# joanrod/star-vector

Measured on AMD Instinct MI355X. Metric: SVG tokens/sec (whole job) + p50 time-to-first-token, StarVector-1B im2svg batch32/GPU, higher is better.
Workload: dtype bf16; 1 GPU; StarVector-1B im2svg, batch 32/GPU, bf16, greedy, 224x224, prompt rows 259 (257 visual + 2), 1024 new tokens/seq, EOS disabled; global_batch=32, parallelism=single, hipgraph_decode=True, decode_steps_per_graph_launch=32, exclusive_device=True

## Files before the change

include/starvector_hip_debug.h:

```cpp
#ifndef STARVECTOR_HIP_DEBUG_H
#define STARVECTOR_HIP_DEBUG_H

#include "starvector_hip.h"

#ifdef __cplusplus
extern "C" {
#endif

int  sv_debug_resample_coeffs(int32_t in_size, int32_t out_size, int32_t* bounds, int32_t* taps, int32_t cap);
int  sv_debug_skinny_plan(int32_t rows, int32_t N, int32_t K, int32_t splitk, int32_t wfmt, int32_t* out2);
enum sv_exp_bits {
    SV_EXP_NO_LN_FOLD        = 2,
    SV_EXP_MLP_FUSED_FORCE   = 128,
    SV_EXP_MLP_FUSED_OFF     = 512,
    SV_EXP_SEPARATE_ARGMAX   = 1024,
    SV_EXP_ROWLN_CATTN_OFF   = 8192,
    SV_EXP_ROWLN_CATTN_FORCE = 16384,
    SV_EXP_NO_PRUNE_LAST     = 32768,
    SV_EXP_BATCH_REMAINDER   = 4194304,
    SV_EXP_KNOWN = SV_EXP_NO_LN_FOLD | SV_EXP_MLP_FUSED_FORCE | SV_EXP_MLP_FUSED_OFF | SV_EXP_SEPARATE_ARGMAX | SV_EXP_ROWLN_CATTN_OFF |
                   SV_EXP_ROWLN_CATTN_FORCE | SV_EXP_NO_PRUNE_LAST | SV_EXP_BATCH_REMAINDER
};
int  sv_debug_set_exp(sv_engine* e, int32_t mask);
int  sv_debug_exp_known(void);
int  sv_debug_gemm_plan(int32_t M, int32_t N, int32_t K, int32_t act, int32_t* out5);
int  sv_debug_decode_plan(int32_t rows, int32_t N, int32_t K, int32_t wfmt, int32_t whole_k, int32_t num_cus, int32_t* out2);
int  sv_debug_attn_plan(int32_t max_batch, int32_t n_kv_head, int32_t num_cus, int32_t* out2);
int  sv_debug_rowln_plan(int32_t D, int32_t N, int32_t splitk, int32_t splitk_ru, int32_t num_cus, int32_t* out3);
int  sv_debug_rowln_occupancy(int32_t wide, int32_t* blocks_per_cu);
int  sv_debug_step_plan(sv_engine* e, int32_t* out4);
int  sv_debug_set_col_tiles(int32_t col_tiles);
int  sv_debug_set_skinny_form(int32_t form);
int  sv_debug_skinny_form(void);
int  sv_debug_tailsplit_launches(int64_t* count);
int  sv_debug_cols_rowhalf_launches(int64_t* launches, int64_t* halves);
int  sv_debug_set_gemm_form(int32_t form);
int  sv_debug_set_linear_seq_rows(int32_t seq_rows);
int  sv_debug_gemm_seq_form(int32_t S, int32_t N, int32_t K, int32_t act);
int  sv_debug_ragged_plan(const int32_t* lens, int32_t B, int32_t N, int32_t K, int32_t act, int32_t q_tile, int32_t* rows_out,
                          int32_t* last_out, int32_t capacity, int32_t* out4);
int  sv_debug_prefix_plan(const int32_t* prefix_lens, int32_t P, const int32_t* lens, const int32_t* prefix_of, int32_t B, int32_t N,
                          int32_t K, int32_t act, int32_t q_tile, int32_t* row_pos_out, int32_t* rows_out, int32_t* blocks_out,
                          int32_t capacity, int32_t* out4);
int  sv_debug_extend_plan(const int32_t* ctx, const int32_t* lens, const int32_t* totals, int32_t B, int32_t budget, int32_t N, int32_t K,
                          int32_t act, int32_t q_tile, int32_t* out, int32_t capacity, int32_t* out_n);
int  sv_debug_shared_plan(const int32_t* lens, int32_t n_prompts, const int32_t* group, const int32_t* budgets, int32_t n,
                          int32_t* shared_out, int32_t* private_out, int64_t* total_out);
int  sv_debug_block_table(sv_engine* e, int32_t row, int32_t* host_out, int32_t capacity);
int  sv_debug_free_pages(sv_engine* e, int32_t* free_out, int32_t* total_out);
int  sv_debug_prompt_passes(sv_engine* e, int64_t* out);
int  sv_debug_attn_trace(sv_engine* e, int64_t* host_out, int32_t capacity_rows);
int  sv_debug_mlp_trace(sv_engine* e, int64_t* host_out, int32_t capacity_blocks);
int  sv_debug_xcc_map(sv_engine* e, int32_t blocks, int32_t heavy, int32_t* host_out);
int  sv_debug_occupy_cus(sv_engine* e, int32_t blocks, int32_t lds_bytes, int32_t ms);
int  sv_debug_gemm_trace(int32_t M, int32_t N, int32_t K, int32_t act, int32_t form, int64_t* host_out, int32_t capacity_blocks);
int  sv_debug_kv_load(sv_engine* e, int32_t layer, const void* dev_kv, int32_t B, int32_t S, const int32_t* dev_lens,
                      sv_stream stream);
int  sv_debug_kv_read(sv_engine* e, int32_t layer, int32_t row, int32_t first, int32_t count, void* dev_out_bf16, sv_stream stream);
int  sv_debug_kv_gather(sv_engine* e, int32_t layer, int32_t row, int32_t count, void* dev_out_bf16, sv_stream stream);
int  sv_debug_page_digests(const void* dev_embeds_packed, int32_t n, const int32_t* host_lens, int32_t S0, int32_t hidden, int32_t max_pages,
                           uint64_t* host_out, sv_stream stream);
int  sv_debug_prefix_hit(const uint64_t* host_digests, int32_t n_pages, int32_t L, const uint64_t* host_table_keys, int32_t n_table,
                         uint64_t* host_keys_out, int32_t* h_out);
int  sv_debug_attn_decode(sv_engine* e, int32_t layer, const float* dev_qkv_f32, int32_t B, void* dev_out, int32_t advance,
                          sv_stream stream);
int  sv_debug_attn_decode_slabs(sv_engine* e, int32_t layer, const float* dev_slabs_f32, int32_t splitk, const void* dev_bias, int32_t B,
                                void* dev_out, int32_t advance, sv_stream stream);
int  sv_debug_attn_decode_draft(sv_engine* e, int32_t layer, const float* dev_slabs_f32, int32_t splitk, const void* dev_bias, int32_t n_seq,
// ... 126 lines not shown
```

star-vector_amd/_lib.py:

```python
from __future__ import annotations

import ctypes as C
import os

HERE = os.path.dirname(os.path.abspath(__file__))
LIB_PATH = os.path.join(HERE, "libstarvector_hip.so")
HEADER_PATH = os.path.normpath(os.path.join(HERE, "..", "include", "starvector_hip.h"))
DEBUG_HEADER_PATH = os.path.normpath(os.path.join(HERE, "..", "include", "starvector_hip_debug.h"))

ABI_VERSION = 9
SV_DTYPE_BF16, SV_DTYPE_F32 = 0, 1
SV_NORM_LAYER, SV_NORM_BATCH = 0, 1
SV_ARCH_V1, SV_ARCH_V2 = 0, 1
ACT = {"none": 0, "quickgelu": 1, "swish": 2, "gelu_tanh": 3}


class SvConfig(C.Structure):
    _fields_ = [
        ("image_size", C.c_int32), ("patch_size", C.c_int32), ("vit_width", C.c_int32),
        ("vit_layers", C.c_int32), ("vit_heads", C.c_int32), ("adapter_norm", C.c_int32),
        ("hidden", C.c_int32), ("n_layer", C.c_int32), ("n_head", C.c_int32), ("n_inner", C.c_int32),
        ("vocab", C.c_int32), ("n_positions", C.c_int32), ("max_batch", C.c_int32),
        ("max_seq_len", C.c_int32), ("ln_eps", C.c_float), ("device", C.c_int32),
        ("arch", C.c_int32), ("n_kv_head", C.c_int32), ("rope_theta", C.c_float), ("vit_mlp", C.c_int32),
# ... 135 lines not shown
    "sv_generate": (_I, [_P, _P, _I, _I, C.POINTER(SvSampling), _P, C.POINTER(_I), _P]),
    "sv_generate_ex": (_I, [_P, _P, _I, _I, C.POINTER(SvSampling), C.POINTER(SvGenerateOutputs), _P, C.POINTER(_I), _P]),
    "sv_cb_admit": (_I, [_P, _P, _I, _I, C.POINTER(SvCbRequest), C.POINTER(_I), _P]),
    "sv_cb_step": (_I, [_P, _I, C.POINTER(_I), _P]),
    "sv_cb_poll": (_I, [_P, C.POINTER(_I), C.POINTER(_I), _I]),
    "sv_cb_read": (_I, [_P, _I, _I, _I, C.POINTER(C.c_int64)]),
    "sv_cb_release": (_I, [_P, _I]),
    "sv_cb_reset": (_I, [_P]),
    "sv_cb_admit_logprobs": (_I, [_P, _P, _I, C.POINTER(_I), _I, C.POINTER(_I), C.POINTER(SvCbRequest), C.POINTER(SvCbLogprobs), C.POINTER(_I), _P]),
    "sv_cb_read_logprobs": (_I, [_P, _I, _I, _I, C.POINTER(_F), C.POINTER(_I), C.POINTER(_I), C.POINTER(_F)]),
    "sv_cb_set_lookup": (_I, [_P, C.POINTER(SvLookup)]),
    "sv_cb_lookup_counts": (_I, [_P, _I, C.POINTER(_I)]),
    "sv_cb_set_prefix_cache": (_I, [_P, _I]),
    "sv_cb_prefix_cache_info": (_I, [_P, C.POINTER(C.c_int64)]),
    "sv_beam_create": (_I, [C.POINTER(SvBeamConfig), C.POINTER(_P)]),
    "sv_beam_destroy": (_I, [_P]),
    "sv_beam_step": (_I, [_P, _P, _I, C.POINTER(_I), C.POINTER(_I), C.POINTER(_I), C.POINTER(_F), _P]),
    "sv_beam_finalize": (_I, [_P, C.POINTER(C.c_int64), C.POINTER(_I), C.POINTER(_F), _P]),
    "sv_beam_history": (_I, [_P, C.POINTER(_I), C.POINTER(_I), _I, C.POINTER(_I), C.POINTER(_I)]),
    "sv_last_timing": (_I, [_P, C.POINTER(C.c_double)]),
}

DEBUG_PROTOTYPES = {
    "sv_debug_resample_coeffs": (_I, [_I, _I, C.POINTER(_I), C.POINTER(_I), _I]),
    "sv_debug_gemm_plan": (_I, [_I, _I, _I, _I, C.POINTER(_I)]),
    "sv_debug_skinny_plan": (_I, [_I, _I, _I, _I, _I, C.POINTER(_I)]),
    "sv_debug_set_exp": (_I, [_P, _I]),
    "sv_debug_exp_known": (_I, []),
    "sv_debug_set_col_tiles": (_I, [_I]),
    "sv_debug_set_skinny_form": (_I, [_I]),
    "sv_debug_skinny_form": (_I, []),
    "sv_debug_tailsplit_launches": (_I, [C.POINTER(C.c_int64)]),
    "sv_debug_cols_rowhalf_launches": (_I, [C.POINTER(C.c_int64), C.POINTER(C.c_int64)]),
    "sv_debug_set_gemm_form": (_I, [_I]),
    "sv_debug_set_linear_seq_rows": (_I, [_I]),
    "sv_debug_gemm_seq_form": (_I, [_I, _I, _I, _I]),
    "sv_debug_ragged_plan": (_I, [C.POINTER(_I), _I, _I, _I, _I, _I, C.POINTER(_I), C.POINTER(_I), _I, C.POINTER(_I)]),
    "sv_debug_prefix_plan": (_I, [C.POINTER(_I), _I, C.POINTER(_I), C.POINTER(_I), _I, _I, _I, _I, _I, C.POINTER(_I), C.POINTER(_I), C.POINTER(_I), _I,
                                  C.POINTER(_I)]),
    "sv_debug_prompt_passes": (_I, [_P, C.POINTER(C.c_int64)]),
    "sv_debug_extend_plan": (_I, [C.POINTER(_I), C.POINTER(_I), C.POINTER(_I), _I, _I, _I, _I, _I, _I, C.POINTER(_I), _I, C.POINTER(_I)]),
    "sv_debug_kv_gather": (_I, [_P, _I, _I, _I, _P, _P]),
    "sv_debug_page_digests": (_I, [_P, _I, C.POINTER(_I), _I, _I, _I, C.POINTER(C.c_uint64), _P]),
    "sv_debug_prefix_hit": (_I, [C.POINTER(C.c_uint64), _I, _I, C.POINTER(C.c_uint64), _I, C.POINTER(C.c_uint64), C.POINTER(_I)]),
    "sv_debug_shared_plan": (_I, [C.POINTER(_I), _I, C.POINTER(_I), C.POINTER(_I), _I, C.POINTER(_I), C.POINTER(_I), C.POINTER(C.c_int64)]),
    "sv_debug_block_table": (_I, [_P, _I, C.POINTER(_I), _I]),
    "sv_debug_free_pages": (_I, [_P, C.POINTER(_I), C.POINTER(_I)]),
    "sv_debug_attn_plan": (_I, [_I, _I, _I, C.POINTER(_I)]),
    "sv_debug_rowln_plan": (_I, [_I, _I, _I, _I, _I, C.POINTER(_I)]),
    "sv_debug_rowln_occupancy": (_I, [_I, C.POINTER(_I)]),
    "sv_debug_step_plan": (_I, [_P, C.POINTER(_I)]),
    "sv_debug_attn_trace": (_I, [_P, C.POINTER(C.c_int64), _I]),
    "sv_debug_mlp_trace": (_I, [_P, C.POINTER(C.c_int64), _I]),
    "sv_debug_xcc_map": (_I, [_P, _I, _I, C.POINTER(_I)]),
    "sv_debug_occupy_cus": (_I, [_P, _I, _I, _I]),
    "sv_debug_gemm_trace": (_I, [_I, _I, _I, _I, _I, C.POINTER(C.c_int64), _I]),
    "sv_debug_kv_load": (_I, [_P, _I, _P, _I, _I, _P, _P]),
    "sv_debug_kv_read": (_I, [_P, _I, _I, _I, _I, _P, _P]),
    "sv_debug_attn_decode": (_I, [_P, _I, _P, _I, _P, _I, _P]),
    "sv_debug_attn_decode_slabs": (_I, [_P, _I, _P, _I, _P, _I, _P, _I, _P]),
    "sv_debug_attn_decode_draft": (_I, [_P, _I, _P, _I, _P, _I, _I, _P, _P]),
    "sv_debug_set_lookup_drafts": (_I, [_P, C.POINTER(_I), _I, _I]),
    "sv_op_lookup_accept": (_I, [C.POINTER(_I), C.POINTER(_I), _I, _I, _I, _I, C.POINTER(_I), _I, C.POINTER(_I), C.POINTER(_I), C.POINTER(_I), _I,
                                 _I, _I, _I, _I, C.POINTER(_I), C.POINTER(_I), _P]),
    "sv_op_lookup_draft": (_I, [C.POINTER(_I), _I, _I, _I, _I, _I, C.POINTER(_I), C.POINTER(_I), _P]),
    "sv_op_lookup_hold": (_I, [_P, _I, _I, _I, _I, _I, C.POINTER(_I), _P]),
# ... 116 lines not shown
```

star-vector_amd/csrc/attention.hip:

```cpp
#include "kernels.h"
#include "kv8/kv8_dev.h"

namespace sv {

__device__ __forceinline__ int swap23(int x) { return (x & ~0xC) | ((x & 4) << 1) | ((x & 8) >> 1); }

template <int D, int HPB, bool RAG = false, bool PFX = false>
__global__ __launch_bounds__(256, 2) void attn_prefill_kernel(AttnPrefillArgs p) {

    constexpr int KSTR = D + 8;
    constexpr int VSTR = 64 + 8;
    constexpr int NKS = D / 16;
    constexpr int NDV = D / 32;
    __shared__ __attribute__((aligned(16))) bf16_t Ks[64 * KSTR];
    __shared__ __attribute__((aligned(16))) bf16_t Vt[D * VSTR];

    const int tid = threadIdx.x, lane = tid & 63;
    const int wave = __builtin_amdgcn_readfirstlane(tid >> 6);
    const int c = lane >> 5;
    int S, qtile;
    size_t row0;
    int pl = 0;
    long long prow = 0, orow = 0;
    if constexpr (PFX) {
// ... 406 lines not shown

template <int D>
struct KvFrags {
    u32x4 k[2][D / 32];
    u32x4 v[D / 16];
};

template <int D>
__device__ __forceinline__ void load_group(KvFrags<D>& f, const char* pool, int page_index, int page_bytes,
                                           int g, int lane) {
    constexpr int NKS = D / 32, NDV = D / 16;
    const int t0 = g << 5;
    const char* page = pool + (size_t)page_index * page_bytes;
    const int half = (t0 >> 5) & 1;
#pragma unroll
    for (int u = 0; u < 2; ++u)
#pragma unroll
        for (int s = 0; s < NKS; ++s)
            f.k[u][s] = *reinterpret_cast<const u32x4*>(page + ((size_t)(((half * 2 + u) * NKS + s) * 64 + lane)) * 16);
#pragma unroll
    for (int t = 0; t < NDV; ++t)
        f.v[t] = *reinterpret_cast<const u32x4*>(page + (size_t)64 * D * 2 + ((size_t)((half * NDV + t) * 64 + lane)) * 16);
}

__device__ __forceinline__ unsigned xcc_id() {
    unsigned x;
    asm volatile("s_getreg_b32 %0, hwreg(HW_REG_XCC_ID)" : "=s"(x));
    return x & 15u;
}

struct AttnDecodeKernarg { const float* ws; const bf16_t* bias; const int32_t* positions; const int32_t* block_table; char* pool_layer;
                           int max_pages; unsigned geom; int ldws; unsigned rows_heads; size_t kv_head_stride; int window;
                           AttnDecodeArgs p; };
template <int D, int NS, int KVF = 0>
__global__ __launch_bounds__(AD_WAVES * 64) void attn_decode_kernel(const float* ws_, const bf16_t* bias_, const int32_t* positions_, const int32_t* block_table_,
                                                                     char* pool_layer_, int max_pages_, unsigned geom_, int ldws_, unsigned rows_heads_,
                                                                     size_t kv_head_stride_, int window_, AttnDecodeArgs p_unused) {
    constexpr int NKS = D / 32;
    constexpr int NDV = D / 16;
    constexpr int PART = 32 + 16 * D;
    const long long t_start = wall_clock64();
    const int n_kv_ = (int)(geom_ & 255u), max_splits_ = (int)((geom_ >> 8) & 255u), gpb_ = (int)((geom_ >> 16) & 255u);
    const int splitk_ = (int)(geom_ >> 24), rows_ws_ = (int)(rows_heads_ & 0xffffu);
    const int H = (int)(rows_heads_ >> 16);
    const int bx = blockIdx.x;
    const int b = bx / n_kv_;
    const int kvh = bx % n_kv_;
    const int split = blockIdx.y;
    const int G = H / n_kv_;
    const int HD = G * D;
    const int tid = threadIdx.x, lane = tid & 63;
    const int wave = __builtin_amdgcn_readfirstlane(tid >> 6);
    const int pos = *reinterpret_cast<const int32_t __attribute__((address_space(4)))*>(reinterpret_cast<uintptr_t>(positions_ + b));

    constexpr int SLT = (AD_WAVES / 2) * 64;
    constexpr int QQ = 16 * D / 4 / SLT;
    static_assert(QQ * SLT * 4 == 16 * D && 2 * D <= SLT && (2 * D & (2 * D - 1)) == 0, "slab work does not tile the upper half of the block");
    const bool slab_wave = wave >= AD_WAVES / 2;
    const unsigned st = (unsigned)tid & (SLT - 1);
    f32x4 sq[QQ][NS];
    float sk[NS];
    uint2 bq[QQ];
    unsigned bk = 0;
    const unsigned kc = st & (2 * D - 1);
    const unsigned kcol = (unsigned)(H * D + kvh * D) + (kc < D ? 0u : (unsigned)(n_kv_ * D)) + (kc & (D - 1));
    auto qcol = [&](int i) -> unsigned {
        const unsigned n = (st + i * SLT) * 4, r = n / D;
// ... 324 lines not shown
                float den = 0.f;
#pragma unroll
                for (int w = 0; w < NWV; ++w) {
                    const float mw = m_s[w * 16 + h];
                    den = fmaf((mw == -INFINITY) ? 0.f : __expf(mw - M), l_s[w * 16 + h], den);
                }
                v[j] = __float_as_uint(is_l ? den : M);
            }
            __builtin_amdgcn_raw_buffer_store_b128(v, rs, my_off + tid * 16, 0, 16);
        }
    };
    if (nwa <= 4) block_merge(std::integral_constant<int, 4>{});
    else if (nwa <= 6) block_merge(std::integral_constant<int, 6>{});
    else block_merge(std::integral_constant<int, AD_WAVES>{});
    auto stamp = [&](long long t_part, long long t_tick, long long t_end) {
        if (p.trace && tid == 0) {
            long long* q = p.trace + ((size_t)bx * gridDim.y + split) * 16;
            q[0] = t_start; q[1] = t_kvreq; q[2] = t_q; q[3] = t_loop; q[4] = t_part; q[5] = t_tick; q[6] = t_end; q[7] = act; q[8] = ngroups;
        }
    };
    if (act == 1) { stamp(0, 0, wall_clock64()); return; }

    asm volatile("s_waitcnt vmcnt(0)" ::: "memory");
    __syncthreads();
    const long long t_part = wall_clock64();
    if (tid == 0) {
        const unsigned t = __hip_atomic_fetch_add(p.counters + bx, 1u, __ATOMIC_RELAXED, __HIP_MEMORY_SCOPE_AGENT);
        flag_s[0] = (t == (unsigned)(act - 1)) ? 1 : 0;
    }
    __syncthreads();
    const long long t_tick = wall_clock64();
    if (!flag_s[0]) { stamp(t_part, t_tick, 0); return; }
    const int seq_off = (int)((size_t)bx * AD_SPLIT * PART * 4);
    for (int idx = tid * 4; idx < HD; idx += AD_WAVES * 64 * 4) {
        const int h = idx / D;
        u32x4 ov[AD_SPLIT];
        float ms[AD_SPLIT], ls[AD_SPLIT];
#pragma unroll
        for (int s2 = 0; s2 < AD_SPLIT; ++s2) {
            ov[s2] = u32x4{0u, 0u, 0u, 0u};
            ms[s2] = -INFINITY; ls[s2] = 0.f;
            if (s2 < act) {
                ms[s2] = __uint_as_float(__builtin_amdgcn_raw_buffer_load_b32(rs, seq_off + (s2 * PART + h) * 4, 0, 16));
                ls[s2] = __uint_as_float(__builtin_amdgcn_raw_buffer_load_b32(rs, seq_off + (s2 * PART + 16 + h) * 4, 0, 16));
                ov[s2] = __builtin_amdgcn_raw_buffer_load_b128(rs, seq_off + (s2 * PART + 32 + idx) * 4, 0, 16);
            }
        }
        float M = -INFINITY;
#pragma unroll
        for (int s2 = 0; s2 < AD_SPLIT; ++s2) M = fmaxf(M, ms[s2]);
        float num[4] = {0.f, 0.f, 0.f, 0.f}, den = 0.f;
#pragma unroll
        for (int s2 = 0; s2 < AD_SPLIT; ++s2) {
            const float f = (s2 < act && ms[s2] != -INFINITY) ? __expf(ms[s2] - M) : 0.f;
            num[0] += f * __uint_as_float(ov[s2][0]); num[1] += f * __uint_as_float(ov[s2][1]);
            num[2] += f * __uint_as_float(ov[s2][2]); num[3] += f * __uint_as_float(ov[s2][3]);
            den += f * ls[s2];
        }
        const float inv = 1.0f / den;
        uint2 o;
        o.x = pack2bf(num[0] * inv, num[1] * inv);
        o.y = pack2bf(num[2] * inv, num[3] * inv);
        *reinterpret_cast<uint2*>(p.out_xp + xp_index(b >> 5, p.out_KS, b & 31, col0 + idx)) = o;
    }
    if (tid == 0) __hip_atomic_store(p.counters + bx, 0u, __ATOMIC_RELAXED, __HIP_MEMORY_SCOPE_AGENT);
    stamp(t_part, t_tick, wall_clock64());
}

size_t attn_decode_part_floats(int head_dim) { return (size_t)AD_SPLIT * (32 + 16 * (size_t)head_dim); }

static size_t attn_decode_smem(int D) {
    return (size_t)(16 * D + 2 * D) * 2 + (size_t)AD_WAVES * 16 * 4 * 2 + (size_t)AD_WAVES * 16 * D * 4 + 16;
}

int init_attention_kernels() {
    const void* k128[4] = {reinterpret_cast<const void*>(&attn_decode_kernel<128, 4>), reinterpret_cast<const void*>(&attn_decode_kernel<128, 8>),
                           reinterpret_cast<const void*>(&attn_decode_kernel<128, 4, 1>), reinterpret_cast<const void*>(&attn_decode_kernel<128, 8, 1>)};
    const void* k64[4] = {reinterpret_cast<const void*>(&attn_decode_kernel<64, 4>), reinterpret_cast<const void*>(&attn_decode_kernel<64, 8>),
                          reinterpret_cast<const void*>(&attn_decode_kernel<64, 4, 1>), reinterpret_cast<const void*>(&attn_decode_kernel<64, 8, 1>)};
    for (int i = 0; i < 4; ++i) {
        hipError_t r = hipFuncSetAttribute(k128[i], hipFuncAttributeMaxDynamicSharedMemorySize, (int)attn_decode_smem(128));
        if (r != hipSuccess) return (int)r;
        r = hipFuncSetAttribute(k64[i], hipFuncAttributeMaxDynamicSharedMemorySize, (int)attn_decode_smem(64));
        if (r != hipSuccess) return (int)r;
    }
    return 0;
}

template <int D, int NS, int KVF = 0>
static void launch_attn_decode_as(const AttnDecodeArgs& a, dim3 grid, size_t smem, hipStream_t st) {
    const int gpb = a.groups_per_block > 0 ? a.groups_per_block : AD_GROUPS_PER_BLOCK;
    const unsigned geom = (unsigned)a.n_kv | (unsigned)grid.y << 8 | (unsigned)gpb << 16 | (unsigned)(a.splitk < 1 ? 1 : a.splitk) << 24;
    const unsigned rows_heads = (unsigned)a.rows_ws | (unsigned)a.H << 16;
    attn_decode_kernel<D, NS, KVF><<<grid, AD_WAVES * 64, smem, st>>>(a.ws, a.bias, a.positions, a.block_table, a.pool_layer, a.max_pages, geom, a.ldws, rows_heads,
                                                                  a.kv_head_stride, a.window, a);
}

void launch_attn_decode(const AttnDecodeArgs& a, hipStream_t st) {
    const size_t smem = attn_decode_smem(a.head_dim);
    dim3 grid(a.B * a.n_kv, a.max_splits < 1 ? 1 : (a.max_splits > AD_SPLIT ? AD_SPLIT : a.max_splits));
    if (a.kv_fmt) {
        if (a.head_dim == 128) {
            if (a.splitk <= 4) launch_attn_decode_as<128, 4, 1>(a, grid, smem, st);
            else launch_attn_decode_as<128, 8, 1>(a, grid, smem, st);
        } else {
            if (a.splitk <= 4) launch_attn_decode_as<64, 4, 1>(a, grid, smem, st);
            else launch_attn_decode_as<64, 8, 1>(a, grid, smem, st);
        }
        return;
    }
    if (a.head_dim == 128) {
        if (a.splitk <= 4) launch_attn_decode_as<128, 4>(a, grid, smem, st);
        else launch_attn_decode_as<128, 8>(a, grid, smem, st);
    } else {
        if (a.splitk <= 4) launch_attn_decode_as<64, 4>(a, grid, smem, st);
        else launch_attn_decode_as<64, 8>(a, grid, smem, st);
    }
}

__global__ __launch_bounds__(AD_WAVES * 64) void xcc_probe_kernel(int32_t* out, int spin_ticks) {
    extern __shared__ __attribute__((aligned(16))) char smem[];
    if (spin_ticks > 0) {
        smem[threadIdx.x] = 1;
        const long long t0 = wall_clock64();
        while (wall_clock64() - t0 < spin_ticks) __builtin_amdgcn_s_sleep(8);
    }
    if (threadIdx.x == 0) out[blockIdx.x] = (int32_t)xcc_id();
}
// ... 24 lines not shown
```

star-vector_amd/csrc/decode_cols.hip:

```cpp
#include "kernels.h"

namespace sv {

struct ColsKernarg { const bf16_t* Wp; const bf16_t* xp; bf16_t* h_xp; const bf16_t* bias; int K, N, cpb, out_KS; ColsArgs p; };

template <int WAVES, int G, int CT, int RH>
__global__ __launch_bounds__(WAVES * 64) void gemm_cols_resid_kernel(const bf16_t* Wp_, const bf16_t* xp_, bf16_t* h_xp_, const bf16_t* bias_,
                                                                     int K_, int N_, int cpb_, int out_KS_, ColsArgs p_unused) {
    static_assert(!RH || CT == 1, "the row-half form is one 16-column tile");
    constexpr int LDT = 16 * CT + 1;
    constexpr int HB = RH ? 1 : 2;
    constexpr int RED = CT * HB * 256;
    extern __shared__ __attribute__((aligned(16))) char dg_smem[];
    float* red = reinterpret_cast<float*>(dg_smem);
    float* tile = red + WAVES * RED;
    const int tid = threadIdx.x, lane = tid & 63;
    const int wave = __builtin_amdgcn_readfirstlane(tid >> 6);
    const int r = lane & 15, g = lane >> 4;
    const int j = blockIdx.x, mt = RH ? 0 : blockIdx.y;
    const int hb0 = RH ? blockIdx.y : 0;
    const int KS = K_ >> 4, C = K_ >> 5;
    const int cpw = (C + WAVES - 1) / WAVES;
    const int c0 = wave * cpw;
    int nc = C - c0;
    nc = nc > cpw ? cpw : nc;
    nc = nc < 0 ? 0 : nc;
    bool wvalid[CT];
    const u32x4* wbase[CT];
#pragma unroll
    for (int t = 0; t < CT; ++t) {
        const int n = j * cpb_ + 16 * t + r;
        wvalid[t] = RH || (16 * t + r < cpb_ && n < N_);
        const int nn = wvalid[t] ? n : 0;
        wbase[t] = reinterpret_cast<const u32x4*>(Wp_) + ((size_t)(nn >> 5) * KS + (g >> 1)) * 64 + (nn & 31) + 32 * (g & 1) + (size_t)c0 * 128;
    }
    const u32x4* xbase = reinterpret_cast<const u32x4*>(xp_) +
                         ((size_t)mt * KS + (g >> 1)) * 64 + 16 * hb0 + r + 32 * (g & 1) + (size_t)c0 * 128;

    f32x4 acc[CT][2];
// ... 1 lines not shown
    for (int t = 0; t < CT; ++t) { acc[t][0] = f32x4{0.f, 0.f, 0.f, 0.f}; acc[t][1] = f32x4{0.f, 0.f, 0.f, 0.f}; }
    const u32x4 zero4 = {0u, 0u, 0u, 0u};
    struct Grp { u32x4 w[CT][G]; u32x4 x[G][HB]; };
    Grp ga, gb;
    auto load = [&](Grp& q, int ci) {
#pragma unroll
        for (int u = 0; u < G; ++u) {
            if (ci + u < nc) {
#pragma unroll
                for (int t = 0; t < CT; ++t) {
                    if constexpr (RH) q.w[t][u] = __builtin_nontemporal_load(wbase[t] + (size_t)(ci + u) * 128);
                    else {
                        q.w[t][u] = zero4;
                        if (wvalid[t]) q.w[t][u] = __builtin_nontemporal_load(wbase[t] + (size_t)(ci + u) * 128);
                    }
                }
                q.x[u][0] = xbase[(size_t)(ci + u) * 128];
                if constexpr (!RH) q.x[u][1] = xbase[(size_t)(ci + u) * 128 + 16];
            }
        }
    };
    auto compute = [&](Grp& q, int ci) {
#pragma unroll
        for (int u = 0; u < G; ++u) {
            if (ci + u < nc) {
#pragma unroll
                for (int t = 0; t < CT; ++t) {
                    acc[t][0] = __builtin_amdgcn_mfma_f32_16x16x32_bf16(as_frag4(q.w[t][u]), as_frag4(q.x[u][0]), acc[t][0], 0, 0, 0);
                    if constexpr (!RH) acc[t][1] = __builtin_amdgcn_mfma_f32_16x16x32_bf16(as_frag4(q.w[t][u]), as_frag4(q.x[u][1]), acc[t][1], 0, 0, 0);
                }
            }
        }
    };
    load(ga, 0);
    if (G < nc) load(gb, G);

    const bool vec = RH || ((cpb_ & 7) == 0 && (N_ & 7) == 0);
    const int v_row = RH ? 16 * hb0 + (tid & 15) : tid & 31, v_ch = RH ? tid >> 4 : tid >> 5;
    const int v_n = j * cpb_ + 8 * v_ch;
    const bool v_on = RH ? tid < 32 : vec && tid < 4 * cpb_ && v_n < N_;
    uint4 v_res = make_uint4(0u, 0u, 0u, 0u), v_bias = make_uint4(0u, 0u, 0u, 0u);
    size_t v_idx = 0;
    const int e_row = tid / cpb_, e_cr = tid - e_row * cpb_;
    const int e_n = j * cpb_ + e_cr;
    const bool e_on = !vec && tid < 32 * cpb_ && e_n < N_;
    float e_bias = 0.f, e_res = 0.f;
    size_t e_idx = 0;
    if (v_on) {
        if (bias_) v_bias = *reinterpret_cast<const uint4*>(bias_ + v_n);
        v_idx = xp_index(mt, out_KS_, v_row, v_n);
        v_res = *reinterpret_cast<const uint4*>(h_xp_ + v_idx);
    }
    if (e_on) {
        if (bias_) e_bias = bf2f(bias_[e_n]);
        e_idx = xp_index(mt, out_KS_, e_row, e_n);
        e_res = bf2f(h_xp_[e_idx]);
    }
    for (int ci = 0; ci < nc; ci += 2 * G) {
        compute(ga, ci);
        if (ci + 2 * G < nc) load(ga, ci + 2 * G);
        if (ci + G < nc) compute(gb, ci + G);
        if (ci + 3 * G < nc) load(gb, ci + 3 * G);
    }

    if (RH || mt == 0) {
        const unsigned pb = RH ? blockIdx.y * gridDim.x + j : j, pn = RH ? gridDim.x * gridDim.y : gridDim.x;
        const ColsArgs pl = sv_late_args<ColsArgs>(offsetof(ColsKernarg, p));
        if (pl.poison) {
            const unsigned share = ((pl.poison_bytes / 16 + pn - 1) / pn) * 16;
            const unsigned lo = pb * share, hi = min(lo + share, pl.poison_bytes);
            const u32x4 ff = {0xffffffffu, 0xffffffffu, 0xffffffffu, 0xffffffffu};
            for (unsigned off = lo + tid * 16; off < hi; off += WAVES * 64 * 16)
                *reinterpret_cast<u32x4*>(reinterpret_cast<char*>(pl.poison) + off) = ff;
        }
        if (pl.poison2) {
            const __amdgpu_buffer_rsrc_t rsp = __builtin_amdgcn_make_buffer_rsrc(pl.poison2, 0, pl.poison2_bytes, 0x00020000);
            const unsigned share = ((pl.poison2_bytes / 16 + pn - 1) / pn) * 16;
            const unsigned lo = pb * share, hi = min(lo + share, pl.poison2_bytes);
            for (unsigned off = lo + tid * 16; off < hi; off += WAVES * 64 * 16)
                __builtin_amdgcn_raw_buffer_store_b128(u32x4{0xffffffffu, 0xffffffffu, 0xffffffffu, 0xffffffffu}, rsp, (int)off, 0, 16);
        }
    }
    {
        float* my = red + wave * RED;
#pragma unroll
        for (int t = 0; t < CT; ++t)
#pragma unroll
            for (int q = 0; q < 4; ++q) {
                my[t * (HB * 256) + q * 64 + lane] = acc[t][0][q];
                if constexpr (!RH) my[t * 512 + (4 + q) * 64 + lane] = acc[t][1][q];
// ... 25 lines not shown

static size_t cols_smem(int waves, int ct) { return (size_t)waves * ct * 512 * 4 + (32 * (16 * ct + 1) + 16) * 4 + 64; }

int cols_pick_cpb(int N, int K) {
    if (K > 2048) {
        int best = 16;
        long best_cost = -1;
        for (int cpb = 8; cpb <= 32; ++cpb) {
            const long nb = (N + cpb - 1) / cpb, rounds = (nb + 255) / 256;
            const long cost = rounds * (cpb + 32);
            if (best_cost < 0 || cost < best_cost) { best_cost = cost; best = cpb; }
        }
        return best;
    }
    int best = 8;
    double best_fill = 0.0;
    for (int cpb = 16; cpb >= 4; cpb >>= 1) {
        const int nb = (N + cpb - 1) / cpb;
        const int rounds = (nb + 255) / 256;
        const double fill = (double)nb / (rounds * 256.0);
        if (fill > best_fill + 1e-9) { best_fill = fill; best = cpb; }
    }
    return best;
}

static size_t cols_smem_rowhalf(int waves) { return (size_t)waves * 256 * 4 + (16 * 17 + 16) * 4 + 64; }

static std::atomic<long long> g_rowhalf_launches{0}, g_rowhalf_halves{0};
void cols_rowhalf_launches(long long* launches, long long* halves) {
    *launches = g_rowhalf_launches.load(std::memory_order_relaxed);
    *halves = g_rowhalf_halves.load(std::memory_order_relaxed);
}

static bool cols_rowhalf(const ColsArgs& a) {
    return a.MT == 1 && a.K <= 2048 && a.N % 16 == 0 && (a.N / 16) % 8 == 0 && env_switch("SV_COLS_ROWHALF", 1);
}

int launch_gemm_cols(const ColsArgs& a, hipStream_t st) {
    if (a.K % 32 || a.cpb < 1 || a.cpb > 32 || !a.h_xp) return -1;
    if (cols_rowhalf(a)) {
        const int halves = (a.M >= 1 && a.M <= 16) ? 1 : 2;
        dim3 grid(a.N / 16, halves);
        gemm_cols_resid_kernel<16, 2, 1, 1><<<grid, 16 * 64, cols_smem_rowhalf(16), st>>>(a.Wp, a.xp, a.h_xp, a.bias, a.K, a.N, 16, a.out_KS, a);
        g_rowhalf_launches.fetch_add(1, std::memory_order_relaxed);
        g_rowhalf_halves.fetch_add(halves, std::memory_order_relaxed);
        return 0;
    }
    dim3 grid((a.N + a.cpb - 1) / a.cpb, a.MT);
    if (a.cpb > 16)
        gemm_cols_resid_kernel<16, 2, 2, 0><<<grid, 16 * 64, cols_smem(16, 2), st>>>(a.Wp, a.xp, a.h_xp, a.bias, a.K, a.N, a.cpb, a.out_KS, a);
    else
        gemm_cols_resid_kernel<16, 2, 1, 0><<<grid, 16 * 64, cols_smem(16, 1), st>>>(a.Wp, a.xp, a.h_xp, a.bias, a.K, a.N, a.cpb, a.out_KS, a);
    return 0;
}

int init_cols_kernels() {
    int r = (int)hipFuncSetAttribute(reinterpret_cast<const void*>(&gemm_cols_resid_kernel<16, 2, 1, 0>),
                                     hipFuncAttributeMaxDynamicSharedMemorySize, (int)cols_smem(16, 1));
    if (!r) r = (int)hipFuncSetAttribute(reinterpret_cast<const void*>(&gemm_cols_resid_kernel<16, 2, 2, 0>),
                                         hipFuncAttributeMaxDynamicSharedMemorySize, (int)cols_smem(16, 2));
    return r;
}

__global__ __launch_bounds__(64) void fold_prepare_kernel(const bf16_t* __restrict__ Wp, const bf16_t* __restrict__ gamma,
                                                          const bf16_t* __restrict__ beta, const bf16_t* __restrict__ bias,
                                                          bf16_t* __restrict__ Wf, float* __restrict__ c1, float* __restrict__ c2, int N, int K) {
    const int nt = blockIdx.x, lane = threadIdx.x;
    const int KS = K >> 4;
    const int n = nt * 32 + (lane & 31), half = lane >> 5;
    float s1 = 0.f, s2 = 0.f;
    for (int ks = 0; ks < KS; ++ks) {
        const size_t off = (((size_t)nt * KS + ks) * 64 + lane) * 8;
        const uint4 wq = *reinterpret_cast<const uint4*>(Wp + off);
        const int k0 = ks * 16 + half * 8;
        const uint4 gq = *reinterpret_cast<const uint4*>(gamma + k0);
        const uint4 bq = *reinterpret_cast<const uint4*>(beta + k0);
// ... 24 lines not shown
```

star-vector_amd/csrc/engine_ops.hip:

```cpp
#include <cmath>
#include "engine_internal.h"

struct TmpBufs {
    std::vector<void*> p;
    ~TmpBufs() { for (void* q : p) (void)hipFree(q); }
    template <typename T> int get(T** out, size_t count) {
        hipError_t r = hipMalloc(reinterpret_cast<void**>(out), count * sizeof(T));
        if (r != hipSuccess) return fail(SV_ENOMEM, "hipMalloc: %s", hipGetErrorString(r));
        p.push_back(*out);
        return 0;
    }
};

extern "C" int sv_debug_set_exp(sv_engine* e, int32_t mask) {
    if (!e) return fail(SV_EINVAL, "null engine");
    SVCHECK(check_exp_mask(mask, "sv_debug_set_exp"));
    std::lock_guard<std::mutex> lk(e->mu);
    e->exp = mask;
    e->xpa_armed = false;
    cb_drop_graphs(e);
    return 0;
}

extern "C" int sv_debug_exp_known(void) { return SV_EXP_KNOWN; }
// ... 439 lines not shown
        return fail(SV_EINVAL, "sv_debug_occupy_cus: blocks 1..4096, lds_bytes 1 KiB..160 KiB, ms 1..5000");
    std::lock_guard<std::mutex> lk(e->mu);
    HIPCHECK(hipSetDevice(e->cfg.device));
    if (!e->tenant_stream) HIPCHECK(hipStreamCreateWithFlags(&e->tenant_stream, hipStreamNonBlocking));
    const int rc = launch_occupy(blocks, lds_bytes, ms * 100000, e->tenant_stream);
    if (rc) return fail(SV_EHIP, "sv_debug_occupy_cus: launch failed (%d)", rc);
    return 0;
}

extern "C" int sv_debug_set_gemm_form(int32_t form) {
    if (form < -1 || form > 3) return fail(SV_EINVAL, "sv_debug_set_gemm_form: -1 (tuned), 0 .. 3");
    set_gemm_form(form);
    return 0;
}

static std::atomic<int> g_op_seq_rows{0};
extern "C" int sv_debug_set_linear_seq_rows(int32_t seq_rows) {
    if (seq_rows < -65536 || seq_rows > 65536) return fail(SV_EINVAL, "sv_debug_set_linear_seq_rows: |S| <= 65536");
    g_op_seq_rows = seq_rows;
    return 0;
}

extern "C" int sv_debug_set_col_tiles(int32_t col_tiles) {
    if (col_tiles < 0 || col_tiles > 3) return fail(SV_EINVAL, "sv_debug_set_col_tiles: 0..3");
    g_op_col_tiles = col_tiles;
    return 0;
}

extern "C" int sv_debug_cols_rowhalf_launches(int64_t* launches, int64_t* halves) {
    if (!launches || !halves) return fail(SV_EINVAL, "sv_debug_cols_rowhalf_launches: null argument");
    long long l = 0, h = 0;
    cols_rowhalf_launches(&l, &h);
    *launches = (int64_t)l; *halves = (int64_t)h;
    return 0;
}
extern "C" int sv_debug_tailsplit_launches(int64_t* count) {
    if (!count) return fail(SV_EINVAL, "sv_debug_tailsplit_launches: null argument");
    *count = (int64_t)tailsplit_launches();
    return 0;
}

extern "C" int sv_debug_set_skinny_form(int32_t form) {
    if (form < 0 || form > 3) return fail(SV_EINVAL, "sv_debug_set_skinny_form: 0..3");
    set_mt2x(form);
    return 0;
}
extern "C" int sv_debug_skinny_form(void) { return get_mt2x(); }

extern "C" int sv_debug_gemm_seq_form(int32_t S, int32_t N, int32_t K, int32_t act) {
    if (S < 1 || N < 1 || K < 1) return fail(SV_EINVAL, "sv_debug_gemm_seq_form: bad argument");
    return gemm_seq_form(S, N, K, act) ? 1 : 0;
}

extern "C" int sv_debug_ragged_plan(const int32_t* lens, int32_t B, int32_t N, int32_t K, int32_t act, int32_t q_tile, int32_t* rows_out,
                                    int32_t* last_out, int32_t capacity, int32_t* out4) {
    if (!lens || !rows_out || !last_out || !out4) return fail(SV_EINVAL, "sv_debug_ragged_plan: null argument");
    if (B < 1 || N < 1 || K < 1 || (q_tile != 32 && q_tile != 128)) return fail(SV_EINVAL, "sv_debug_ragged_plan: bad argument (B %d, N %d, K %d, q_tile %d)", B, N, K, q_tile);
    if (capacity < 3 * B) return fail(SV_EINVAL, "sv_debug_ragged_plan: capacity %d < 3 * B", capacity);
    for (int b = 0; b < B; ++b)
        if (lens[b] < 1) return fail(SV_EINVAL, "sv_debug_ragged_plan: length %d of sequence %d", lens[b], b);
    PackedPlan pp;
    const PlanProj pj{N, K, act};
    ragged_plan(lens, B, q_tile, &pj, 1, nullptr, pp);
    std::copy(pp.rows(0).begin(), pp.rows(0).end(), rows_out);
    std::copy(pp.last(0).begin(), pp.last(0).end(), last_out);
    out4[0] = (int32_t)pp.rows(0).size(); out4[1] = (int32_t)pp.last(0).size();
// ... 1348 lines not shown
```

star-vector_amd/csrc/kernels.h:

```cpp
#pragma once
#include <hip/hip_runtime.h>
#include <stdint.h>
#include <stdlib.h>
#include <atomic>
#include "common.h"

namespace sv {

inline int round_up(int a, int b) { return (a + b - 1) / b * b; }
inline int env_switch(const char* name, int dflt) {
    const char* ev = getenv(name);
    return ev ? atoi(ev) : dflt;
}

void launch_pack_weight(const void* src, int src_is_f32, bf16_t* dst, int N, int K, int Npad, int Kpad,
                        hipStream_t st);
void launch_convert_to_bf16(const void* src, int src_is_f32, bf16_t* dst, size_t n, hipStream_t st);
void launch_pack_weight_fp8(const void* src, int src_is_f32, bf16_t* dst_bf16, uint8_t* dst_q, float* scale, int N, int K,
                            int Npad, int Kpad, hipStream_t st);
enum { SV_WFMT_BF16 = 0, SV_WFMT_FP8 = 1, SV_WFMT_MXFP4 = 2 };
#define SV_MXFP4_GROUP 1088
inline size_t mxfp4_image_bytes(int Npad, int Kpad) { return (size_t)(Npad / 32) * (Kpad / 64) * SV_MXFP4_GROUP; }
void launch_pack_weight_mxfp4(const void* src, int src_is_f32, bf16_t* dst_bf16, uint8_t* dst_w4, uint8_t* scale_plain, int N, int K,
                              int Npad, int Kpad, hipStream_t st);
// ... 73 lines not shown
extern std::atomic<int> g_op_col_tiles;

int init_gemm_kernels();

void launch_cvt_bf16_hw(const float* x, bf16_t* y, size_t n, hipStream_t st);

struct MlpFusedArgs {
    const bf16_t* W1; const bf16_t* x1;
    int N1, N1pad, K1;
    const float* fold_c1; const float* fold_c2; int fold_D; float fold_eps; int act;
    bf16_t* out_xp; int out_KS;
    const bf16_t* W2; int N2, N2pad, K2;
    int splitk;
    float* ws; int ldws; int rows_ws;
    int* err;
    int spin_ticks;
    long long* trace;
};
int launch_mlp_fused(const MlpFusedArgs& a, hipStream_t st);

struct ColsArgs {
    const bf16_t* xp;
    const bf16_t* Wp;
    const bf16_t* bias;
    int MT, N, K;
    int M;
    int cpb;
    bf16_t* h_xp; int out_KS;
    void* poison; unsigned poison_bytes;
    void* poison2; unsigned poison2_bytes;
};
int cols_pick_cpb(int N, int K);
int launch_gemm_cols(const ColsArgs& a, hipStream_t st);
void cols_rowhalf_launches(long long* launches, long long* halves);
int init_cols_kernels();
void launch_fold_prepare(const bf16_t* Wp, const bf16_t* gamma, const bf16_t* beta, const bf16_t* bias, bf16_t* Wf, float* c1, float* c2,
                         int N, int Npad, int K, hipStream_t st);

void launch_layernorm_rows(const bf16_t* x, int ldx, const bf16_t* g, const bf16_t* b, bf16_t* y, int ldy,
                           int M, int D, float eps, hipStream_t st);
void launch_layernorm_rows_packed(const bf16_t* x, int ldx, const bf16_t* g, const bf16_t* b, bf16_t* yp,
                                  int M, int D, float eps, hipStream_t st);

struct RowUpdateArgs {
    const float* ws; int splitk; int ldws; int rows_ws;
    const bf16_t* bias;
    bf16_t* h; int ldh;
    const bf16_t* wte; const bf16_t* wpe;
    const int32_t* tokens; const int32_t* positions;
    const bf16_t* g; const bf16_t* b; float eps;
    bf16_t* xp_out;
    int M, D;
};
void launch_row_update_ln(const RowUpdateArgs& a, hipStream_t st);
struct RowCattnArgs {
    const bf16_t* g; const bf16_t* b; float eps; int D;
    const bf16_t* wte; const bf16_t* wpe; const int32_t* tokens; const int32_t* positions;
    bf16_t* xp_out;
    float* ws_out; int ldws_out;
    int* err; int spin_ticks;
    int delay;
    int first_round;
    int ldh;
    long long* dbg; int layer;
};
int launch_rowln_cattn(const RowUpdateArgs& ru, const SkinnyArgs& sk, int* err, int spin_ticks, hipStream_t st, int delay = 390, long long* dbg = nullptr, int layer = 0,
// ... 381 lines not shown
```

star-vector_amd/engine.py:

```python
from __future__ import annotations

import ctypes as C
import enum
import os
import threading
from dataclasses import dataclass
from typing import Dict, Iterable, List, NamedTuple, Optional, Sequence, Tuple

import torch

from . import _lib
from ._lib import SvConfig, SvSampling, check


class Exp(enum.IntFlag):
    NO_LN_FOLD = 2
    MLP_FUSED_FORCE = 128
    MLP_FUSED_OFF = 512
    SEPARATE_ARGMAX = 1024
    ROWLN_CATTN_OFF = 8192
    ROWLN_CATTN_FORCE = 16384
    NO_PRUNE_LAST = 32768
    BATCH_REMAINDER = 4194304

# ... 1218 lines not shown

def shared_plan(lengths: Sequence[int], group: Sequence[int], budgets: Sequence[int]) -> Dict[str, object]:
    U, n = len(lengths), len(group)
    sh, pv, tot = (C.c_int32 * max(n, 1))(), (C.c_int32 * max(n, 1))(), C.c_int64(0)
    check(_lib.load().sv_debug_shared_plan((C.c_int32 * max(U, 1))(*[int(v) for v in lengths]), U, (C.c_int32 * max(n, 1))(*[int(v) for v in group]),
                                           (C.c_int32 * max(n, 1))(*[int(v) for v in budgets]), n, sh, pv, C.byref(tot)), "sv_debug_shared_plan")
    return {"shared": list(sh)[:n], "private": list(pv)[:n], "total": int(tot.value)}


def set_skinny_form(form: int) -> None:
    check(_lib.load().sv_debug_set_skinny_form(int(form)))


def skinny_form() -> int:
    return int(_lib.load().sv_debug_skinny_form())


def set_op_col_tiles(col_tiles: int) -> None:
    check(_lib.load().sv_debug_set_col_tiles(int(col_tiles)))


def tailsplit_launches() -> int:
    n = C.c_int64(0)
    check(_lib.load().sv_debug_tailsplit_launches(C.byref(n)), "sv_debug_tailsplit_launches")
    return n.value


def cols_rowhalf_launches() -> tuple[int, int]:
    n, h = C.c_int64(0), C.c_int64(0)
    check(_lib.load().sv_debug_cols_rowhalf_launches(C.byref(n), C.byref(h)), "sv_debug_cols_rowhalf_launches")
    return n.value, h.value


def op_linear_skinny(x, W, bias=None, splitk=1):
    lib = _lib.load()
    x = _need(x, torch.bfloat16, "x"); W = _need(W, torch.bfloat16, "W")
    M, K = x.shape; N = W.shape[0]
    y = torch.empty(M, N, dtype=torch.float32, device=x.device)
    b = _need(bias, torch.bfloat16, "bias") if bias is not None else None
    check(lib.sv_op_linear_skinny(_ptr(x), _ptr(W), _ptr(b), _ptr(y), M, N, K, splitk, _stream()))
    return y


def op_linear_skinny_fp8(x, W, bias=None, splitk=1):
    lib = _lib.load()
    x = _need(x, torch.bfloat16, "x"); W = _need(W, torch.bfloat16, "W")
    M, K = x.shape; N = W.shape[0]
    y = torch.empty(M, N, dtype=torch.float32, device=x.device)
    sc = torch.empty(N, dtype=torch.float32, device=x.device)
    b = _need(bias, torch.bfloat16, "bias") if bias is not None else None
    check(lib.sv_op_linear_skinny_fp8(_ptr(x), _ptr(W), _ptr(b), _ptr(y), _ptr(sc), M, N, K, splitk, _stream()))
    return y, sc


def op_linear_skinny_epi(x, W, bias=None, act="none", out_f32=False):
    lib = _lib.load()
    x = _need(x, torch.bfloat16, "x"); W = _need(W, torch.bfloat16, "W")
    M, K = x.shape; N = W.shape[0]
    y = torch.empty(M, N, dtype=torch.float32 if out_f32 else torch.bfloat16, device=x.device)
    b = _need(bias, torch.bfloat16, "bias") if bias is not None else None
    check(lib.sv_op_linear_skinny_epi(_ptr(x), _ptr(W), _ptr(b), _ptr(y), M, N, K, _lib.ACT[act], int(out_f32), _stream()),
          "sv_op_linear_skinny_epi")
    return y


def op_linear_skinny_epi_fp8(x, W, bias=None, act="none", out_f32=False):
# ... 788 lines not shown
```

Baseline: 32360 tokens/s.

## Stage attention split-merge stats in LDS and add single-pass cols GEMM path

Attention decode gains a merge variant where wave 0 loads the per-split max/sum statistics into LDS while the other waves issue their partial-output loads, followed by one barrier and a compile-time unrolled merge, with a short specialization for at most 8 active splits. The row-half cols GEMM gains an XW form that, when the K range exactly fits two load groups, issues all x and weight loads up front and runs the MFMAs without the double-buffered loop. Both are on by default behind env switches and come with debug launch counters. The goal is to cut load latency and loop overhead in small decode kernels, at the cost of extra kernel instantiations and more registers held live.

```diff
diff --git a/include/starvector_hip_debug.h b/include/starvector_hip_debug.h
--- a/include/starvector_hip_debug.h
+++ b/include/starvector_hip_debug.h
@@ -34,6 +34,8 @@
 int  sv_debug_skinny_form(void);
 int  sv_debug_tailsplit_launches(int64_t* count);
 int  sv_debug_cols_rowhalf_launches(int64_t* launches, int64_t* halves);
+int  sv_debug_attn_merge_lds_launches(int64_t* count);
+int  sv_debug_cols_xw_launches(int64_t* count);
 int  sv_debug_set_gemm_form(int32_t form);
 int  sv_debug_set_linear_seq_rows(int32_t seq_rows);
 int  sv_debug_gemm_seq_form(int32_t S, int32_t N, int32_t K, int32_t act);
diff --git a/star-vector_amd/_lib.py b/star-vector_amd/_lib.py
--- a/star-vector_amd/_lib.py
+++ b/star-vector_amd/_lib.py
@@ -191,6 +191,8 @@
     "sv_debug_skinny_form": (_I, []),
     "sv_debug_tailsplit_launches": (_I, [C.POINTER(C.c_int64)]),
     "sv_debug_cols_rowhalf_launches": (_I, [C.POINTER(C.c_int64), C.POINTER(C.c_int64)]),
+    "sv_debug_attn_merge_lds_launches": (_I, [C.POINTER(C.c_int64)]),
+    "sv_debug_cols_xw_launches": (_I, [C.POINTER(C.c_int64)]),
     "sv_debug_set_gemm_form": (_I, [_I]),
     "sv_debug_set_linear_seq_rows": (_I, [_I]),
     "sv_debug_gemm_seq_form": (_I, [_I, _I, _I, _I]),
diff --git a/star-vector_amd/csrc/attention.hip b/star-vector_amd/csrc/attention.hip
--- a/star-vector_amd/csrc/attention.hip
+++ b/star-vector_amd/csrc/attention.hip
@@ -462,7 +462,7 @@
 struct AttnDecodeKernarg { const float* ws; const bf16_t* bias; const int32_t* positions; const int32_t* block_table; char* pool_layer;
                            int max_pages; unsigned geom; int ldws; unsigned rows_heads; size_t kv_head_stride; int window;
                            AttnDecodeArgs p; };
-template <int D, int NS, int KVF = 0>
+template <int D, int NS, int KVF = 0, int MLDS = 1>
 __global__ __launch_bounds__(AD_WAVES * 64) void attn_decode_kernel(const float* ws_, const bf16_t* bias_, const int32_t* positions_, const int32_t* block_table_,
                                                                      char* pool_layer_, int max_pages_, unsigned geom_, int ldws_, unsigned rows_heads_,
                                                                      size_t kv_head_stride_, int window_, AttnDecodeArgs p_unused) {
@@ -853,6 +853,74 @@
     const long long t_tick = wall_clock64();
     if (!flag_s[0]) { stamp(t_part, t_tick, 0); return; }
     const int seq_off = (int)((size_t)bx * AD_SPLIT * PART * 4);
+    if constexpr (MLDS != 0) {
+        float* st_s = O_s;
+        const int idx = tid * 4;
+        const bool on = idx < HD;
+        const int idc = on ? idx : 0;
+        const bool wave_on = wave * 256 < HD;
+        const int h = idc / D;
+        const int actu = __builtin_amdgcn_readfirstlane(act);
+        auto merge = [&](auto nb_tag) {
+            constexpr int NB = decltype(nb_tag)::value;
+            u32x4 ov[NB], sv[NB / 8];
+            auto o_issue = [&]() {
+#pragma unroll
+                for (int s2 = 0; s2 < NB; ++s2)
+                    ov[s2] = __builtin_amdgcn_raw_buffer_load_b128(rs, seq_off + (32 + idc) * 4, (s2 < actu ? s2 : actu - 1) * (PART * 4), 16);
+            };
+            if (wave == 0) {
+#pragma unroll
+                for (int j = 0; j < NB / 8; ++j) {
+                    const int pc = j * 64 + lane, s2 = pc >> 3;
+                    sv[j] = __builtin_amdgcn_raw_buffer_load_b128(rs, seq_off + ((s2 < actu ? s2 : actu - 1) * PART + (pc & 7) * 4) * 4, 0, 16);
+                }
+                o_issue();
+#pragma unroll
+                for (int j = 0; j < NB / 8; ++j) {
+                    asm volatile("" : "+v"(sv[j]));
+                    *reinterpret_cast<u32x4*>(st_s + (j * 64 + lane) * 4) = sv[j];
+                }
+                asm volatile("; statistics in LDS" ::: "memory");
+            } else if (wave_on) {
+                o_issue();
+                asm volatile("; O requested" ::: "memory");
+            } else {
+#pragma unroll
+                for (int s2 = 0; s2 < NB; ++s2) ov[s2] = u32x4{0u, 0u, 0u, 0u};
+            }
+            __syncthreads();
+            float ms[NB], ls[NB];
+#pragma unroll
+            for (int s2 = 0; s2 < NB; ++s2) {
+                const float mv = st_s[s2 * 32 + h], lv = st_s[s2 * 32 + 16 + h];
+                ms[s2] = s2 < actu ? mv : -INFINITY;
+                ls[s2] = s2 < actu ? lv : 0.f;
+            }
+            float M = -INFINITY;
+#pragma unroll
+            for (int s2 = 0; s2 < NB; ++s2) M = fmaxf(M, ms[s2]);
+            float num[4] = {0.f, 0.f, 0.f, 0.f}, den = 0.f;
+#pragma unroll
+            for (int s2 = 0; s2 < NB; ++s2) {
+                const float f = (s2 < actu && ms[s2] != -INFINITY) ? __expf(ms[s2] - M) : 0.f;
+                asm volatile("" : "+v"(ov[s2]));
+                const u32x4 o = s2 < actu ? ov[s2] : u32x4{0u, 0u, 0u, 0u};
+                num[0] = fmaf(f, __uint_as_float(o[0]), num[0]); num[1] = fmaf(f, __uint_as_float(o[1]), num[1]);
+                num[2] = fmaf(f, __uint_as_float(o[2]), num[2]); num[3] = fmaf(f, __uint_as_float(o[3]), num[3]);
+                den = fmaf(f, ls[s2], den);
+            }
+            if (on) {
+                const float inv = 1.0f / den;
+                uint2 o;
+                o.x = pack2bf(num[0] * inv, num[1] * inv);
+                o.y = pack2bf(num[2] * inv, num[3] * inv);
+                *reinterpret_cast<uint2*>(p.out_xp + xp_index(b >> 5, p.out_KS, b & 31, col0 + idx)) = o;
+            }
+        };
+        if (actu <= 8) merge(std::integral_constant<int, 8>{});
+        else merge(std::integral_constant<int, AD_SPLIT>{});
+    } else
     for (int idx = tid * 4; idx < HD; idx += AD_WAVES * 64 * 4) {
         const int h = idx / D;
         u32x4 ov[AD_SPLIT];
@@ -894,11 +962,12 @@
     return (size_t)(16 * D + 2 * D) * 2 + (size_t)AD_WAVES * 16 * 4 * 2 + (size_t)AD_WAVES * 16 * D * 4 + 16;
 }
 
-int init_attention_kernels() {
-    const void* k128[4] = {reinterpret_cast<const void*>(&attn_decode_kernel<128, 4>), reinterpret_cast<const void*>(&attn_decode_kernel<128, 8>),
-                           reinterpret_cast<const void*>(&attn_decode_kernel<128, 4, 1>), reinterpret_cast<const void*>(&attn_decode_kernel<128, 8, 1>)};
-    const void* k64[4] = {reinterpret_cast<const void*>(&attn_decode_kernel<64, 4>), reinterpret_cast<const void*>(&attn_decode_kernel<64, 8>),
-                          reinterpret_cast<const void*>(&attn_decode_kernel<64, 4, 1>), reinterpret_cast<const void*>(&attn_decode_kernel<64, 8, 1>)};
+template <int MLDS>
+static int init_attention_kernels_as() {
+    const void* k128[4] = {reinterpret_cast<const void*>(&attn_decode_kernel<128, 4, 0, MLDS>), reinterpret_cast<const void*>(&attn_decode_kernel<128, 8, 0, MLDS>),
+                           reinterpret_cast<const void*>(&attn_decode_kernel<128, 4, 1, MLDS>), reinterpret_cast<const void*>(&attn_decode_kernel<128, 8, 1, MLDS>)};
+    const void* k64[4] = {reinterpret_cast<const void*>(&attn_decode_kernel<64, 4, 0, MLDS>), reinterpret_cast<const void*>(&attn_decode_kernel<64, 8, 0, MLDS>),
+                          reinterpret_cast<const void*>(&attn_decode_kernel<64, 4, 1, MLDS>), reinterpret_cast<const void*>(&attn_decode_kernel<64, 8, 1, MLDS>)};
     for (int i = 0; i < 4; ++i) {
         hipError_t r = hipFuncSetAttribute(k128[i], hipFuncAttributeMaxDynamicSharedMemorySize, (int)attn_decode_smem(128));
         if (r != hipSuccess) return (int)r;
@@ -907,14 +976,28 @@
     }
     return 0;
 }
-
-template <int D, int NS, int KVF = 0>
-static void launch_attn_decode_as(const AttnDecodeArgs& a, dim3 grid, size_t smem, hipStream_t st) {
+int init_attention_kernels() {
+    const int r = init_attention_kernels_as<0>();
+    return r ? r : init_attention_kernels_as<1>();
+}
+
+template <int D, int NS, int KVF, int MLDS>
+static void launch_attn_decode_form(const AttnDecodeArgs& a, dim3 grid, size_t smem, hipStream_t st) {
     const int gpb = a.groups_per_block > 0 ? a.groups_per_block : AD_GROUPS_PER_BLOCK;
     const unsigned geom = (unsigned)a.n_kv | (unsigned)grid.y << 8 | (unsigned)gpb << 16 | (unsigned)(a.splitk < 1 ? 1 : a.splitk) << 24;
     const unsigned rows_heads = (unsigned)a.rows_ws | (unsigned)a.H << 16;
-    attn_decode_kernel<D, NS, KVF><<<grid, AD_WAVES * 64, smem, st>>>(a.ws, a.bias, a.positions, a.block_table, a.pool_layer, a.max_pages, geom, a.ldws, rows_heads,
-                                                                  a.kv_head_stride, a.window, a);
+    attn_decode_kernel<D, NS, KVF, MLDS><<<grid, AD_WAVES * 64, smem, st>>>(a.ws, a.bias, a.positions, a.block_table, a.pool_layer, a.max_pages, geom, a.ldws, rows_heads,
+                                                                       a.kv_head_stride, a.window, a);
+}
+
+static std::atomic<long long> g_merge_lds_launches{0};
+long long attn_merge_lds_launches() { return g_merge_lds_launches.load(std::memory_order_relaxed); }
+template <int D, int NS, int KVF = 0>
+static void launch_attn_decode_as(const AttnDecodeArgs& a, dim3 grid, size_t smem, hipStream_t st) {
+    if (env_switch("SV_ATTN_MERGE_LDS", 1)) {
+        launch_attn_decode_form<D, NS, KVF, 1>(a, grid, smem, st);
+        g_merge_lds_launches.fetch_add(1, std::memory_order_relaxed);
+    } else launch_attn_decode_form<D, NS, KVF, 0>(a, grid, smem, st);
 }
 
 void launch_attn_decode(const AttnDecodeArgs& a, hipStream_t st) {
diff --git a/star-vector_amd/csrc/decode_cols.hip b/star-vector_amd/csrc/decode_cols.hip
--- a/star-vector_amd/csrc/decode_cols.hip
+++ b/star-vector_amd/csrc/decode_cols.hip
@@ -4,7 +4,7 @@
 
 struct ColsKernarg { const bf16_t* Wp; const bf16_t* xp; bf16_t* h_xp; const bf16_t* bias; int K, N, cpb, out_KS; ColsArgs p; };
 
-template <int WAVES, int G, int CT, int RH>
+template <int WAVES, int G, int CT, int RH, int XW = 0>
 __global__ __launch_bounds__(WAVES * 64) void gemm_cols_resid_kernel(const bf16_t* Wp_, const bf16_t* xp_, bf16_t* h_xp_, const bf16_t* bias_,
                                                                      int K_, int N_, int cpb_, int out_KS_, ColsArgs p_unused) {
     static_assert(!RH || CT == 1, "the row-half form is one 16-column tile");
@@ -72,8 +72,21 @@
             }
         }
     };
-    load(ga, 0);
-    if (G < nc) load(gb, G);
+    bool fit = false;
+    if constexpr (RH && XW != 0) fit = C == WAVES * 2 * G;
+    if (fit) {
+#pragma unroll
+        for (int u = 0; u < G; ++u) ga.x[u][0] = xbase[(size_t)u * 128];
+#pragma unroll
+        for (int u = 0; u < G; ++u) gb.x[u][0] = xbase[(size_t)(G + u) * 128];
+#pragma unroll
+        for (int u = 0; u < G; ++u) ga.w[0][u] = __builtin_nontemporal_load(wbase[0] + (size_t)u * 128);
+#pragma unroll
+        for (int u = 0; u < G; ++u) gb.w[0][u] = __builtin_nontemporal_load(wbase[0] + (size_t)(G + u) * 128);
+    } else {
+        load(ga, 0);
+        if (G < nc) load(gb, G);
+    }
 
     const bool vec = RH || ((cpb_ & 7) == 0 && (N_ & 7) == 0);
     const int v_row = RH ? 16 * hb0 + (tid & 15) : tid & 31, v_ch = RH ? tid >> 4 : tid >> 5;
@@ -96,6 +109,12 @@
         e_idx = xp_index(mt, out_KS_, e_row, e_n);
         e_res = bf2f(h_xp_[e_idx]);
     }
+    if (fit) {
+#pragma unroll
+        for (int u = 0; u < G; ++u) acc[0][0] = __builtin_amdgcn_mfma_f32_16x16x32_bf16(as_frag4(ga.w[0][u]), as_frag4(ga.x[u][0]), acc[0][0], 0, 0, 0);
+#pragma unroll
+        for (int u = 0; u < G; ++u) acc[0][0] = __builtin_amdgcn_mfma_f32_16x16x32_bf16(as_frag4(gb.w[0][u]), as_frag4(gb.x[u][0]), acc[0][0], 0, 0, 0);
+    } else
     for (int ci = 0; ci < nc; ci += 2 * G) {
         compute(ga, ci);
         if (ci + 2 * G < nc) load(ga, ci + 2 * G);
@@ -187,6 +206,8 @@
     *halves = g_rowhalf_halves.load(std::memory_order_relaxed);
 }
 
+static std::atomic<long long> g_cols_xw_launches{0};
+long long cols_xw_launches() { return g_cols_xw_launches.load(std::memory_order_relaxed); }
 static bool cols_rowhalf(const ColsArgs& a) {
     return a.MT == 1 && a.K <= 2048 && a.N % 16 == 0 && (a.N / 16) % 8 == 0 && env_switch("SV_COLS_ROWHALF", 1);
 }
@@ -196,7 +217,10 @@
     if (cols_rowhalf(a)) {
         const int halves = (a.M >= 1 && a.M <= 16) ? 1 : 2;
         dim3 grid(a.N / 16, halves);
-        gemm_cols_resid_kernel<16, 2, 1, 1><<<grid, 16 * 64, cols_smem_rowhalf(16), st>>>(a.Wp, a.xp, a.h_xp, a.bias, a.K, a.N, 16, a.out_KS, a);
+        if (env_switch("SV_COLS_XW", 1)) {
+            gemm_cols_resid_kernel<16, 2, 1, 1, 1><<<grid, 16 * 64, cols_smem_rowhalf(16), st>>>(a.Wp, a.xp, a.h_xp, a.bias, a.K, a.N, 16, a.out_KS, a);
+            g_cols_xw_launches.fetch_add(1, std::memory_order_relaxed);
+        } else gemm_cols_resid_kernel<16, 2, 1, 1><<<grid, 16 * 64, cols_smem_rowhalf(16), st>>>(a.Wp, a.xp, a.h_xp, a.bias, a.K, a.N, 16, a.out_KS, a);
         g_rowhalf_launches.fetch_add(1, std::memory_order_relaxed);
         g_rowhalf_halves.fetch_add(halves, std::memory_order_relaxed);
         return 0;
diff --git a/star-vector_amd/csrc/engine_ops.hip b/star-vector_amd/csrc/engine_ops.hip
--- a/star-vector_amd/csrc/engine_ops.hip
+++ b/star-vector_amd/csrc/engine_ops.hip
@@ -495,6 +495,16 @@
     long long l = 0, h = 0;
     cols_rowhalf_launches(&l, &h);
     *launches = (int64_t)l; *halves = (int64_t)h;
+    return 0;
+}
+extern "C" int sv_debug_attn_merge_lds_launches(int64_t* count) {
+    if (!count) return fail(SV_EINVAL, "sv_debug_attn_merge_lds_launches: null argument");
+    *count = (int64_t)attn_merge_lds_launches();
+    return 0;
+}
+extern "C" int sv_debug_cols_xw_launches(int64_t* count) {
+    if (!count) return fail(SV_EINVAL, "sv_debug_cols_xw_launches: null argument");
+    *count = (int64_t)cols_xw_launches();
     return 0;
 }
 extern "C" int sv_debug_tailsplit_launches(int64_t* count) {
diff --git a/star-vector_amd/csrc/kernels.h b/star-vector_amd/csrc/kernels.h
--- a/star-vector_amd/csrc/kernels.h
+++ b/star-vector_amd/csrc/kernels.h
@@ -129,6 +129,8 @@
 };
 int cols_pick_cpb(int N, int K);
 int launch_gemm_cols(const ColsArgs& a, hipStream_t st);
+long long attn_merge_lds_launches();
+long long cols_xw_launches();
 void cols_rowhalf_launches(long long* launches, long long* halves);
 int init_cols_kernels();
 void launch_fold_prepare(const bf16_t* Wp, const bf16_t* gamma, const bf16_t* beta, const bf16_t* bias, bf16_t* Wf, float* c1, float* c2,
diff --git a/star-vector_amd/engine.py b/star-vector_amd/engine.py
--- a/star-vector_amd/engine.py
+++ b/star-vector_amd/engine.py
@@ -1274,6 +1274,18 @@
     return n.value, h.value
 
 
+def cols_xw_launches() -> int:
+    n = C.c_int64(0)
+    check(_lib.load().sv_debug_cols_xw_launches(C.byref(n)), "sv_debug_cols_xw_launches")
+    return n.value
+
+
+def attn_merge_lds_launches() -> int:
+    n = C.c_int64(0)
+    check(_lib.load().sv_debug_attn_merge_lds_launches(C.byref(n)), "sv_debug_attn_merge_lds_launches")
+    return n.value
+
+
 def op_linear_skinny(x, W, bias=None, splitk=1):
     lib = _lib.load()
     x = _need(x, torch.bfloat16, "x"); W = _need(W, torch.bfloat16, "W")
```

New measurement: 32590 tokens/s, median of 6. No clear change (+0.7%).
